# ironhide23586/RoomNet

Hardware: AMD Instinct MI355X
Metric: images/sec, 224x224 batch-256 RoomNet inference (higher is better)
Workload: dtype bf16; 1 GPU; RoomNet forward (reference final_model weights), uint8 BGR 224x224x3 in HBM -> probs+ids in HBM, batch 256 per GPU, bf16 storage / fp32 accumulate; images_per_gpu=256, global_batch=256, im_side=224, parallelism=dp1

## Files before the change

roomnet_amd/csrc/rn_fused.hip:

```cpp
#include "rn_fused.h"
#include <map>
#include <vector>
#include <algorithm>
#include <atomic>
#include "rn_stage.h"

#include <cmath>
#include <cstring>
#include <cstdlib>

using namespace rnk;

namespace {

constexpr int S0_CO = 8;
constexpr int S0_TSTRIDE = 29;
constexpr int S0_AHEAD = 8;

struct Stage0Args {
    const uint8_t* bgr;
    const i32x4* wfrag;
    const float* ptab;
    unsigned short* out;
    int S, So;
// ... 1123 lines not shown
            for (int b = 1; b <= 8 && b <= max_bands; ++b) {
                const long rounds = (per_band * b + n_cu - 1) / n_cu;
                const long cost = rounds * ((s2.out_side + b - 1) / b + 11);
                if (best_cost < 0 || cost < best_cost) {
                    best_cost = cost;
                    bands = b;
                }
            }
            if (per_band * bands < n_cu) {
                bands = static_cast<int>((n_cu + per_band - 1) / per_band);
                if (bands > max_bands) bands = max_bands;
            }
            fa.rows_per_band = (s2.out_side + bands - 1) / bands;
            fa.n_bands = (s2.out_side + fa.rows_per_band - 1) / fa.rows_per_band;
#ifdef RN_STAMPS
            static unsigned long long* stamp_host23 = nullptr;
            const size_t nwaves23 = static_cast<size_t>(fa.n_bands) * fa.n_cblocks * n * 8;
            if (!stamp_host23) (void)hipHostMalloc(reinterpret_cast<void**>(&stamp_host23), 16u << 20, 0);
            std::memset(stamp_host23, 0, nwaves23 * 96);
            fa.stamp_buf = stamp_host23;
#endif
#ifdef RN_CLOCK
            if (fs->pair_x16) fa.stamp_buf = rn_clock_region("stages 2+3", static_cast<size_t>(fa.n_bands) * fa.n_cblocks * n);
#endif
#ifdef RN_ROUND2_ARMS
            int rc = fs->pair_x16 ? rn_stage23x_launch(h->dtype, h->stream, fa, n) : rn_stage23_launch(h->dtype, h->stream, fa, n);
#else
            int rc = rn_stage23x_launch(h->dtype, h->stream, fa, n);
#endif
            if (rc != RN_OK) return rc;
#ifdef RN_STAMPS
            (void)hipStreamSynchronize(h->stream);
            {
                double wtot[8] = {0}, wbar[8] = {0}, wsteps[8] = {0};
                for (size_t k = 0; k < nwaves23; ++k) {
                    wtot[k & 7] += stamp_host23[k * 4];
                    wbar[k & 7] += stamp_host23[k * 4 + 2];
                    wsteps[k & 7] += stamp_host23[k * 4 + 3];
                }
                {
                    double seg[2][6] = {{0}, {0}};
                    double st[2] = {0, 0};
                    const unsigned long long* base = stamp_host23 + nwaves23 * 4;
                    for (size_t k = 0; k < nwaves23; ++k) {
                        const int role = (k & 7) < 4 ? 0 : 1;
                        st[role] += stamp_host23[k * 4 + 3];
                        for (int j = 0; j < 6; ++j) seg[role][j] += base[k * 8 + j];
                    }
                    fprintf(stderr, "[stamps]   producer segments (chain0 epi0 chain1 epi1): %.0f %.0f %.0f %.0f\n", seg[0][0] / st[0], seg[0][1] / st[0],
                            seg[0][2] / st[0], seg[0][3] / st[0]);
                    fprintf(stderr, "[stamps]   consumer segments (bookkeeping+own-fetch chain0 skip-wait epi0 chain1+epi1): %.0f %.0f %.0f %.0f %.0f\n", seg[1][0] / st[1],
                            seg[1][2] / st[1], seg[1][3] / st[1], seg[1][4] / st[1], seg[1][5] / st[1]);
                }
                for (int w8 = 0; w8 < 8; ++w8)
                    if (wsteps[w8] > 0)
                        fprintf(stderr, "[stamps] fused stages %zu+%zu wave %d (%s): cycles/step %.0f, of which barrier wait %.0f\n", i, i + 1, w8,
                                w8 < 4 ? "producer" : "consumer", wtot[w8] / wsteps[w8], wbar[w8] / wsteps[w8]);
            }
#endif
            rn_record_event(h, 2 + static_cast<int>(i) + 1);
            ++i;
            continue;
        }
        StageArgs a{};
        a.in = static_cast<const unsigned short*>(h->nodes[prev.node_bn2 >= 0 ? prev.node_bn2 : prev.node_bn].ptr);
        a.out = static_cast<unsigned short*>(h->nodes[s.node_bn2 >= 0 ? s.node_bn2 : s.node_bn].ptr);
        a.wfrag = f.wfrag;
        a.bn_mean = s.bn.mean;
        a.bn_inv = s.bn.inv;
        a.bn_beta = s.bn.beta;
        if (s.skip_stage >= 0) {
            const StagePlan& sk = h->stages[s.skip_stage];
            if (sk.node_bn2 >= 0) {
                rn_set_error("16-bit path: skip source with its own residual is not supported");
                return RN_E_INVALID;
            }
            a.skip = static_cast<const unsigned short*>(h->nodes[sk.node_bn].ptr);
            a.bn2_mean = s.bn2.mean;
            a.bn2_inv = s.bn2.inv;
            a.bn2_beta = s.bn2.beta;
            a.rlo = s.rt.lo;
            a.rhi = s.rt.hi;
            a.rlerp = s.rt.lerp;
            a.Ss = s.skip_side;
            a.rscale = static_cast<float>(s.skip_side) / static_cast<float>(s.out_side);
        }
        a.H = a.W = s.in_side;
        a.Ho = a.Wo = s.out_side;
        a.dither = fs->dither_out[i];
        a.plain_q = -1;
// ... 277 lines not shown
```

roomnet_amd/csrc/rn_stage23x.hip:

```cpp
#include "rn_fused.h"
#include "rn_stage.h"

#include <atomic>
#include <utility>

using namespace rnk;

namespace {

template <int DT>
__device__ __forceinline__ unsigned pack2p(float a, float b) {
    return pack2<DT>(a, b);
}

constexpr int RN_NT_OUT = 2, RN_NT_SKIP = 2;
constexpr int X_NA = 4, X_NB = 4, X_NSK = 3;
constexpr int X_WMIN = 193;
constexpr int X_WMAX = 215;
constexpr int X_ROWA = X_WMAX * 64;
constexpr int X_BDUMMY = X_WMAX - 5;
constexpr int X_ROWB = (X_BDUMMY + 1) * 64;
constexpr int X_SKROW = 64 * 64;
constexpr int X_ROWB_N = (X_BDUMMY + 1) * 32;
constexpr int X_ROWB_8 = (X_BDUMMY + 1) * 16;
constexpr int X_NTAB = 6 * 32;
constexpr int X_RINGA_OFF = 1024;
constexpr int X_RINGB_OFF = X_RINGA_OFF + X_NA * X_ROWA;
constexpr int X_SKIP_OFF = X_RINGB_OFF + X_NB * X_ROWB;
constexpr int X_LDS = X_SKIP_OFF + 4 * X_NSK * X_SKROW;
constexpr int X_LAG = 11;
constexpr int X_KT = 9;
static_assert(X_LDS <= 160 * 1024, "LDS budget");

__device__ __forceinline__ int xp_start(int w) { return w == 0 ? 0 : w == 1 ? 61 : w == 2 ? 122 : 167; }
__device__ __forceinline__ int xc_start(int w) { return w == 0 ? 0 : w == 1 ? 45 : w == 2 ? 90 : 148; }

__device__ __forceinline__ unsigned lds_addr(const void* p) {
    return static_cast<unsigned>(reinterpret_cast<uintptr_t>((__attribute__((address_space(3))) const char*)p));
}

__device__ __forceinline__ int swzx(int pix) { return (pix >> 1) & 3; }

using i32x2 = __attribute__((ext_vector_type(2))) int;

template <int DT>
__device__ __forceinline__ f32x4 mfma16(i32x4 a, i32x4 b, f32x4 c) {
    if constexpr (DT == RN_DTYPE_BF16)
        return __builtin_amdgcn_mfma_f32_16x16x32_bf16(__builtin_bit_cast(bf16x8, a), __builtin_bit_cast(bf16x8, b), c, 0, 0, 0);
    else
        return __builtin_amdgcn_mfma_f32_16x16x32_f16(__builtin_bit_cast(f16x8, a), __builtin_bit_cast(f16x8, b), c, 0, 0, 0);
}

template <int DT, int PH, bool NB, bool N8 = false>
__global__ __launch_bounds__(512, 2) void stage23x_kernel(const Stage23Args a) {
    static_assert(!NB || PH == 1, "the narrow B ring holds the computed half only");
    static_assert(!N8 || NB, "the eight-channel ring is a narrow ring");
    constexpr int ROWB = N8 ? X_ROWB_8 : NB ? X_ROWB_N : X_ROWB;
    constexpr int AHEAD = 3;
    extern __shared__ __attribute__((aligned(64))) char smem[];
    const int tid = threadIdx.x;
    const int lane = tid & 63;
    const int wave = __builtin_amdgcn_readfirstlane(tid >> 6);
    const int wq = wave & 3;
    const int px16 = lane & 15, g = lane >> 4;
#ifdef RN_CLOCK
    unsigned long long ck_t0, ck_r0;
    clock_pair(ck_t0, ck_r0);
#endif
    const int cblk = blockIdx.x % a.n_cblocks, band = blockIdx.x / a.n_cblocks, n = blockIdx.y;
    const int Win = a.W, Hout = a.Wo, x0 = a.cb_x0[cblk];
    const int Wo = a.cb_wo[cblk], W = Wo + 10, Wb = W - 5;
    const int yo0 = band * a.rows_per_band;
    const int nrows = min(Hout, yo0 + a.rows_per_band) - yo0;
    const int nsteps = nrows + X_LAG;

    float* const tab = reinterpret_cast<float*>(smem);
    for (int i = tid; i < X_NTAB; i += 512) tab[i] = a.ptab[i];
    char* const ringA = smem + X_RINGA_OFF;
    char* const ringB = smem + X_RINGB_OFF;
    const unsigned ringA_lds = lds_addr(ringA), ringB_lds = lds_addr(ringB);
    const char* const in_img = reinterpret_cast<const char*>(a.in + static_cast<int64_t>(n) * Win * Win * 32);
    const char* const in_blk = in_img + x0 * 64;
    constexpr int OOB = 0x40000000;
    const f32x4 zero4 = {0.f, 0.f, 0.f, 0.f};

    i32x4 pm, pmx;
#pragma unroll
    for (int d = 0; d < 4; ++d) {
        unsigned w0 = 0, w1 = 0;
#pragma unroll
        for (int e2 = 0; e2 < 2; ++e2) {
            const int e = 2 * d + e2;
            const int p = 4 * g + (e & 3);
            w0 |= ((p >= px16 && p < px16 + 4) ? 0x3C00u : 0u) << (16 * e2);
            w1 |= ((16 + p >= px16 && 16 + p < px16 + 4) ? 0x3C00u : 0u) << (16 * e2);
        }
        pm[d] = static_cast<int>(w0);
        pmx[d] = static_cast<int>(w1);
    }
    asm volatile("" : "+v"(pm), "+v"(pmx));

    auto chain = [&](auto S0C, auto ROWC, auto KC, const unsigned (&base)[3], const i32x4 (&wr)[2 * X_KT], f32x4 (&acc)[2], auto&& hook) __attribute__((always_inline)) {
        constexpr int S0 = decltype(S0C)::value, ROW = decltype(ROWC)::value, k = decltype(KC)::value;
        i32x4 fq[X_KT];
        auto rd = [&](auto TC, float dep) __attribute__((always_inline)) -> i32x4 {
            constexpr int tap = decltype(TC)::value, ky = tap / 3, kx = tap % 3;
            constexpr int off = ((S0 + ky) % 4) * ROW + k * 1024;
            i32x4 v;
            asm volatile("ds_read_b128 %0, %1 offset:%2" : "=v"(v) : "v"(base[kx]), "n"(off), "v"(dep));
            return v;
        };
        [&]<int... I>(std::integer_sequence<int, I...>) { ((fq[I] = rd(IC<I>{}, 0.f)), ...); }(std::make_integer_sequence<int, AHEAD>{});
// ... 17 lines not shown
        if constexpr (sub == 1) vt[h][1] = static_cast<int>(pack2_relu6_sixth(acc[h][2], acc[h][3]));
        if constexpr (sub == 2) {
            const int n0 = pk_add_f16(hp[h][0], vt[h][0]), n1 = pk_add_f16(hp[h][1], vt[h][1]);
            hp[h][0] = vt[h][0];
            hp[h][1] = vt[h][1];
            if constexpr (NB) {
                auto& Q = PR == 0 ? q0[h] : q1[h];
                Q[2 * HI] = n0;
                Q[2 * HI + 1] = n1;
                op[h] = Q;
            } else {
                auto& qold = PR == 0 ? q0[h] : q1[h];
                op[h] = i32x4{qold[0], qold[1], n0, n1};
                qold[0] = n0;
                qold[1] = n1;
            }
        }
    };
    auto finish = [&](auto PRC, const f32x4 (&acc)[2], int (&hp)[2][2], auto& q0, auto& q1, i32x4 (&op)[2]) __attribute__((always_inline)) {
        int vt[2][2];
        [&]<int... I>(std::integer_sequence<int, I...>) { (finish_part(IC<I>{}, PRC, acc, hp, q0, q1, op, vt), ...); }(std::make_integer_sequence<int, 6>{});
    };
    auto with_finish = [&](auto&& base, auto PRC, const f32x4 (&acc)[2], int (&hp)[2][2], auto& q0, auto& q1, i32x4 (&op)[2],
                           int (&vt)[2][2]) __attribute__((always_inline)) {
        return [&, PRC](auto IC_) __attribute__((always_inline)) {
            constexpr int i = decltype(IC_)::value;
            base(IC_);
            if constexpr (i >= 1 && i <= 6) finish_part(IC<(i >= 1 && i <= 6 ? i - 1 : 0)>{}, PRC, acc, hp, q0, q1, op, vt);
        };
    };

    const int xs0 = a.rlo[x0 + min(xc_start(wq), Wo - 1)];
    const unsigned sk_goff0 = static_cast<unsigned>((xs0 + (lane >> 2)) * 64 + ((lane & 3) << 4));
    char* const skw = smem + X_SKIP_OFF + wq * (X_NSK * X_SKROW);
    const unsigned skw_lds = lds_addr(skw);
    auto issue_skip_piece = [&](auto IC_, int y, int slot) __attribute__((always_inline)) {
        constexpr int i = decltype(IC_)::value;
        const char* row = in_img + static_cast<int64_t>(y) * static_cast<int64_t>(Win * 64);
        unsigned off = sk_goff0;
        asm volatile("" : "+v"(off));
        __builtin_amdgcn_global_load_lds(row + i * 1024 + off, (lds_void_ptr)(skw + slot * X_SKROW + i * 1024), 16, 0, RN_NT_SKIP);
    };
    auto issue_skip_row = [&](int y, int slot) __attribute__((always_inline)) {
        issue_skip_piece(IC<0>{}, y, slot);
        issue_skip_piece(IC<1>{}, y, slot);
        issue_skip_piece(IC<2>{}, y, slot);
        issue_skip_piece(IC<3>{}, y, slot);
    };
    auto no_hook = [](auto) __attribute__((always_inline)) {};
    struct VLerp {
        int ylo;
        float yl;
    };
    auto vlerp_of = [&](int yo) __attribute__((always_inline)) -> VLerp {
        const float src = mul_rounded(static_cast<float>(yo), a.rscale);
        const int ylo = static_cast<int>(src);
        VLerp v;
        v.ylo = __builtin_amdgcn_readfirstlane(ylo);
        v.yl = __int_as_float(__builtin_amdgcn_readfirstlane(__float_as_int(src - static_cast<float>(ylo))));
        return v;
    };
    int sk_f = vlerp_of(yo0).ylo - 1;
    int sk_slot = X_NSK - 1;
    auto ylo_step = [&](int t) __attribute__((always_inline)) {
        return vlerp_of(yo0 + min(max(t - X_LAG, 0), nrows - 1)).ylo;
    };

// ... 46 lines not shown
        for (int k = 0; k < 4; ++k) {
            const int xo = xw + 16 * k + px16;
            const bool last = k == (has4 ? 3 : 2);
            const int col = (xo < Wb && !(last && px16 >= 13) && (k < 3 || has4)) ? xo : X_BDUMMY;
            if constexpr (N8)
                wbB[k] = ringB_lds + static_cast<unsigned>((g < 2 ? col : X_BDUMMY) * 16 + 8 * (g & 1));
            else if constexpr (NB)
                wbB[k] = ringB_lds + static_cast<unsigned>(col * 32 + 8 * g);
            else
                wbB[k] = ringB_lds + static_cast<unsigned>(col * 64 + ((g ^ swzx(col)) << 4));
        }
        f32x4 scv[2], shv[2];
#pragma unroll
        for (int h = 0; h < 2; ++h) {
            scv[h] = *reinterpret_cast<const f32x4*>(a.ptab + 8 * g + 4 * h);
            shv[h] = *reinterpret_cast<const f32x4*>(a.ptab + 32 + 8 * g + 4 * h);
        }
        int hp[4][2][2];
        std::conditional_t<NB, i32x4[4][2], int[4][2][2]> q0, q1;
#pragma unroll
        for (int k = 0; k < 4; ++k)
#pragma unroll
            for (int h = 0; h < 2; ++h)
#pragma unroll
                for (int j = 0; j < 2; ++j) {
                    hp[k][h][j] = 0;
                    if constexpr (NB) {
                        q0[k][h][2 * j] = q0[k][h][2 * j + 1] = q1[k][h][2 * j] = q1[k][h][2 * j + 1] = 0;
                    } else {
                        q0[k][h][j] = q1[k][h][j] = 0;
                    }
                }
        issue_A_pieces(a_next, 0);
        int ylo_nxt = ylo_step(0);
        wait_vmcnt<0>();
#pragma unroll
        for (int f = 0; f < 2 * X_KT; ++f)
            if (PH == 2 || !(f & 1)) asm volatile("" : "+v"(w2[f]));
        lds_barrier();
        [[maybe_unused]] const int cdead0 = static_cast<int>(pack2p<DT>(shv[1][0], shv[1][1])), cdead1 = static_cast<int>(pack2p<DT>(shv[1][2], shv[1][3]));

        [[maybe_unused]] auto chain2 = [&](auto S0C, auto K0C, auto K1C, f32x4& acc0, f32x4& acc1, auto&& hook) __attribute__((always_inline)) {
            constexpr int S0 = decltype(S0C)::value, k0 = decltype(K0C)::value, k1 = decltype(K1C)::value;
            i32x4 fa[X_KT], fb[X_KT];
            auto rd = [&](auto TC, auto KC_, float dep) __attribute__((always_inline)) -> i32x4 {
                constexpr int tap = decltype(TC)::value, ky = tap / 3, kx = tap % 3, k = decltype(KC_)::value;
                constexpr int off = ((S0 + ky) % 4) * X_ROWA + k * 1024;
                i32x4 v;
                asm volatile("ds_read_b128 %0, %1 offset:%2" : "=v"(v) : "v"(baseA[kx]), "n"(off), "v"(dep));
                return v;
            };
            [&]<int... I>(std::integer_sequence<int, I...>) { ((fa[I] = rd(IC<I>{}, IC<k0>{}, 0.f), fb[I] = rd(IC<I>{}, IC<k1>{}, 0.f)), ...); }(std::make_integer_sequence<int, AHEAD>{});
            [&]<int... I>(std::integer_sequence<int, I...>) {
                (([&] {
                     if constexpr (I + AHEAD < X_KT) {
                         fa[I + AHEAD] = rd(IC<(I + AHEAD < X_KT ? I + AHEAD : 0)>{}, IC<k0>{}, I == 0 ? 0.f : acc0[0]);
                         fb[I + AHEAD] = rd(IC<(I + AHEAD < X_KT ? I + AHEAD : 0)>{}, IC<k1>{}, I == 0 ? 0.f : acc1[0]);
                     }
                     constexpr int newer = (X_KT - 1 - I) < AHEAD ? (X_KT - 1 - I) : AHEAD;
                     asm volatile("s_waitcnt lgkmcnt(%2)" : "+v"(fa[I]), "+v"(fb[I]) : "n"(2 * newer));
                     acc0 = mfma16<DT>(fa[I], w2[2 * I], I == 0 ? zero4 : acc0);
                     acc1 = mfma16<DT>(fb[I], w2[2 * I], I == 0 ? zero4 : acc1);
                     hook(IC<I>{});
                 }()),
                 ...);
            }(std::make_integer_sequence<int, X_KT>{});
        };
        [[maybe_unused]] auto chain1 = [&](auto S0C, auto KC_, f32x4& acc0, auto&& hook) __attribute__((always_inline)) {
            constexpr int S0 = decltype(S0C)::value, k = decltype(KC_)::value;
            i32x4 fa[X_KT];
            auto rd = [&](auto TC, float dep) __attribute__((always_inline)) -> i32x4 {
                constexpr int tap = decltype(TC)::value, ky = tap / 3, kx = tap % 3;
                constexpr int off = ((S0 + ky) % 4) * X_ROWA + k * 1024;
                i32x4 v;
                asm volatile("ds_read_b128 %0, %1 offset:%2" : "=v"(v) : "v"(baseA[kx]), "n"(off), "v"(dep));
                return v;
            };
            [&]<int... I>(std::integer_sequence<int, I...>) { ((fa[I] = rd(IC<I>{}, 0.f)), ...); }(std::make_integer_sequence<int, AHEAD>{});
            [&]<int... I>(std::integer_sequence<int, I...>) {
                (([&] {
                     if constexpr (I + AHEAD < X_KT) fa[I + AHEAD] = rd(IC<(I + AHEAD < X_KT ? I + AHEAD : 0)>{}, I == 0 ? 0.f : acc0[0]);
                     constexpr int newer = (X_KT - 1 - I) < AHEAD ? (X_KT - 1 - I) : AHEAD;
                     asm volatile("s_waitcnt lgkmcnt(%1)" : "+v"(fa[I]) : "n"(newer));
                     acc0 = mfma16<DT>(fa[I], w2[2 * I], I == 0 ? zero4 : acc0);
                     hook(IC<I>{});
                 }()),
                 ...);
            }(std::make_integer_sequence<int, X_KT>{});
        };
        [[maybe_unused]] auto with_finish2 = [&](auto&& base, auto PRC, const f32x4 (&accx)[2], int (&hpx)[2][2], auto& q0x, auto& q1x, i32x4 (&opx)[2],
                                const f32x4 (&accy)[2], int (&hpy)[2][2], auto& q0y, auto& q1y, i32x4 (&opy)[2], int (&vt)[2][2]) __attribute__((always_inline)) {
            return [&, PRC](auto IC_) __attribute__((always_inline)) {
                constexpr int i = decltype(IC_)::value;
                base(IC_);
                if constexpr (i >= 1 && i <= 3) finish_part(IC<(i >= 1 && i <= 3 ? i - 1 : 0)>{}, PRC, accx, hpx, q0x, q1x, opx, vt);
                if constexpr (i >= 4 && i <= 6) finish_part(IC<(i >= 4 && i <= 6 ? i - 4 : 0)>{}, PRC, accy, hpy, q0y, q1y, opy, vt);
            };
        };
        [[maybe_unused]] auto finish1 = [&](auto PRC, const f32x4 (&acc)[2], int (&hpx)[2][2], auto& q0x, auto& q1x, i32x4 (&opx)[2]) __attribute__((always_inline)) {
            int vt[2][2];
            finish_part(IC<0>{}, PRC, acc, hpx, q0x, q1x, opx, vt);
            finish_part(IC<1>{}, PRC, acc, hpx, q0x, q1x, opx, vt);
            finish_part(IC<2>{}, PRC, acc, hpx, q0x, q1x, opx, vt);
        };
        [[maybe_unused]] auto out1 = [&](auto KC, auto PC, const i32x4 (&opk)[2], const i32x4 (&opn)[2], bool cross) __attribute__((always_inline)) {
            constexpr int k = decltype(KC)::value, P = decltype(PC)::value;
            constexpr int off = ((P + 3) % X_NB) * ROWB;
            f32x4 H = mfma16<RN_DTYPE_F16>(opk[0], pm, zero4);
// ... 1 lines not shown
            float y[4];
#pragma unroll
            for (int i = 0; i < 4; ++i) y[i] = __builtin_fmaf(H[i], scv[0][i], shv[0][i]);
            auto& wb = wbB;
            if constexpr (NB) {
                const i32x2 d = {static_cast<int>(pack2p<DT>(y[0], y[1])), static_cast<int>(pack2p<DT>(y[2], y[3]))};
                asm volatile("ds_write_b64 %0, %1 offset:%2" ::"v"(wb[k]), "v"(d), "n"(off) : "memory");
            } else {
                const i32x4 d = {static_cast<int>(pack2p<DT>(y[0], y[1])), static_cast<int>(pack2p<DT>(y[2], y[3])), cdead0, cdead1};
                asm volatile("ds_write_b128 %0, %1 offset:%2" ::"v"(wb[k]), "v"(d), "n"(off) : "memory");
            }
        };

        auto out = [&](auto KC, auto PC, const i32x4 (&opk)[2], const i32x4 (&opn)[2], bool cross) __attribute__((always_inline)) {
            constexpr int k = decltype(KC)::value, P = decltype(PC)::value;
            constexpr int off = ((P + 3) % X_NB) * X_ROWB;
            f32x4 H[2];
#pragma unroll
            for (int h = 0; h < 2; ++h) H[h] = mfma16<RN_DTYPE_F16>(opk[h], pm, zero4);
            if (cross) {
#pragma unroll
                for (int h = 0; h < 2; ++h) H[h] = mfma16<RN_DTYPE_F16>(opn[h], pmx, H[h]);
            }
            float y[8];
#pragma unroll
            for (int h = 0; h < 2; ++h)
#pragma unroll
                for (int i = 0; i < 4; ++i) y[4 * h + i] = __builtin_fmaf(H[h][i], scv[h][i], shv[h][i]);
            const i32x4 d = {static_cast<int>(pack2p<DT>(y[0], y[1])), static_cast<int>(pack2p<DT>(y[2], y[3])),
                             static_cast<int>(pack2p<DT>(y[4], y[5])), static_cast<int>(pack2p<DT>(y[6], y[7]))};
            auto& wb = wbB;
            asm volatile("ds_write_b128 %0, %1 offset:%2" ::"v"(wb[k]), "v"(d), "n"(off) : "memory");
        };
        auto step = [&](auto PC, int t) __attribute__((always_inline)) {
            constexpr int P = decltype(PC)::value;
            [[maybe_unused]] constexpr int PR = P & 1;
            if (t < nrows + 9) a_next += Win * 64;
            auto hook0 = [&](auto IC_) __attribute__((always_inline)) {
                constexpr int i = decltype(IC_)::value;
                if constexpr (i == 1) issue_A_piece(IC<0>{}, a_next, (P + 1) % X_NA);
                if constexpr (i == 5) issue_A_piece(IC<1>{}, a_next, (P + 1) % X_NA);
                if constexpr (i == 3) {
                    const int need_cur = min(ylo_nxt + 1, Win - 1);
                    if (sk_f < need_cur) {
                        ++sk_f;
                        sk_slot = sk_slot == X_NSK - 1 ? 0 : sk_slot + 1;
                    }
                }
                if constexpr (i == 7) {
                    ylo_nxt = ylo_step(t + 1);
                    const int need_next = min(ylo_nxt + 1, Win - 1);
                    if (sk_f < need_next) {
                        ++sk_f;
                        sk_slot = sk_slot == X_NSK - 1 ? 0 : sk_slot + 1;
                    }
                }
            };
            auto hook1 = [&](auto IC_) __attribute__((always_inline)) {
                constexpr int i = decltype(IC_)::value;
                if constexpr (i == 1) issue_A_piece(IC<2>{}, a_next, (P + 1) % X_NA);
                if constexpr (i == 5) issue_A_piece(IC<3>{}, a_next, (P + 1) % X_NA);
            };
            auto hook2 = [&](auto IC_) __attribute__((always_inline)) {
                constexpr int i = decltype(IC_)::value;
                if constexpr (i == 0) issue_skip_piece(IC<0>{}, sk_f, sk_slot);
                if constexpr (i == 2) issue_skip_piece(IC<1>{}, sk_f, sk_slot);
                if constexpr (i == 4) issue_skip_piece(IC<2>{}, sk_f, sk_slot);
                if constexpr (i == 6) issue_skip_piece(IC<3>{}, sk_f, sk_slot);
            };
            if constexpr (PH == 1) {
                auto hookA = [&](auto IC_) __attribute__((always_inline)) {
                    constexpr int i = decltype(IC_)::value;
                    if constexpr (i == 0) issue_A_piece(IC<0>{}, a_next, (P + 1) % X_NA);
                    if constexpr (i == 2) issue_A_piece(IC<1>{}, a_next, (P + 1) % X_NA);
                    if constexpr (i == 4) issue_A_piece(IC<2>{}, a_next, (P + 1) % X_NA);
                    if constexpr (i == 6) issue_A_piece(IC<3>{}, a_next, (P + 1) % X_NA);
                    if constexpr (i == 3 || i == 7) hook0(IC_);
                };
                f32x4 ac0[2], ac1[2], ac2[2], ac3[2];
                int vt[2][2];
                i32x4 op[4][2];
                op[3][0] = op[3][1] = i32x4{0, 0, 0, 0};
                chain2(IC<(P + 2) % 4>{}, IC<0>{}, IC<1>{}, ac0[0], ac1[0], hookA);
                if (has4) {
                    chain2(IC<(P + 2) % 4>{}, IC<2>{}, IC<3>{}, ac2[0], ac3[0],
                           with_finish2(hook2, IC<(P & 3)>{}, ac0, hp[0], q0[0], q1[0], op[0], ac1, hp[1], q0[1], q1[1], op[1], vt));
                    out1(IC<0>{}, PC, op[0], op[1], true);
                    finish1(IC<(P & 3)>{}, ac2, hp[2], q0[2], q1[2], op[2]);
                    out1(IC<1>{}, PC, op[1], op[2], true);
                    finish1(IC<(P & 3)>{}, ac3, hp[3], q0[3], q1[3], op[3]);
                    out1(IC<2>{}, PC, op[2], op[3], true);
                    out1(IC<3>{}, PC, op[3], op[3], false);
                } else {
                    chain1(IC<(P + 2) % 4>{}, IC<2>{}, ac2[0],
                           with_finish2(hook2, IC<(P & 3)>{}, ac0, hp[0], q0[0], q1[0], op[0], ac1, hp[1], q0[1], q1[1], op[1], vt));
                    out1(IC<0>{}, PC, op[0], op[1], true);
                    finish1(IC<(P & 3)>{}, ac2, hp[2], q0[2], q1[2], op[2]);
                    out1(IC<1>{}, PC, op[1], op[2], true);
                    out1(IC<2>{}, PC, op[2], op[3], true);
                }
                wait_vmcnt<0>();
                asm volatile("s_waitcnt lgkmcnt(0)" ::: "memory");
                raw_barrier();
                return;
            }
            f32x4 accA[2], accB[2];
            int vt[2][2];
            i32x4 op[4][2];
            op[3][0] = op[3][1] = i32x4{0, 0, 0, 0};
            chain(IC<(P + 2) % 4>{}, IC<X_ROWA>{}, IC<0>{}, baseA, w2, accA, hook0);
            chain(IC<(P + 2) % 4>{}, IC<X_ROWA>{}, IC<1>{}, baseA, w2, accB, with_finish(hook1, IC<(P & 3)>{}, accA, hp[0], q0[0], q1[0], op[0], vt));
            chain(IC<(P + 2) % 4>{}, IC<X_ROWA>{}, IC<2>{}, baseA, w2, accA, with_finish(hook2, IC<(P & 3)>{}, accB, hp[1], q0[1], q1[1], op[1], vt));
            out(IC<0>{}, PC, op[0], op[1], true);
            if (has4) {
                chain(IC<(P + 2) % 4>{}, IC<X_ROWA>{}, IC<3>{}, baseA, w2, accB, with_finish(no_hook, IC<(P & 3)>{}, accA, hp[2], q0[2], q1[2], op[2], vt));
                out(IC<1>{}, PC, op[1], op[2], true);
                finish(IC<(P & 3)>{}, accB, hp[3], q0[3], q1[3], op[3]);
                out(IC<2>{}, PC, op[2], op[3], true);
                out(IC<3>{}, PC, op[3], op[3], false);
            } else {
                finish(IC<(P & 3)>{}, accA, hp[2], q0[2], q1[2], op[2]);
                out(IC<1>{}, PC, op[1], op[2], true);
                out(IC<2>{}, PC, op[2], op[3], true);
            }
            wait_vmcnt<0>();
            asm volatile("s_waitcnt lgkmcnt(0)" ::: "memory");
            raw_barrier();
        };
        int t = 0;
        for (; t + 3 < nsteps; t += 4) {
            step(IC<0>{}, t);
            step(IC<1>{}, t + 1);
            step(IC<2>{}, t + 2);
            step(IC<3>{}, t + 3);
        }
        const int rem = nsteps - t;
        if (rem > 0) step(IC<0>{}, t);
        if (rem > 1) step(IC<1>{}, t + 1);
        if (rem > 2) step(IC<2>{}, t + 2);
        wait_vmcnt<0>();
        return;
    }

    __builtin_amdgcn_s_setprio(1);
    const bool has4 = wq >= 2;
    const int xw = xc_start(wq);
    const int xend = wq == 3 ? Wo : min(xc_start(wq + 1), Wo);
    constexpr int NW3 = N8 ? 6 : NB ? 10 : 2 * X_KT;
    i32x4 w3[2 * X_KT];
#pragma unroll
    for (int f = 0; f < NW3; ++f) {
        const i32x4* src = a.wfrag3 + f * 64 + lane;
        asm volatile("global_load_dwordx4 %0, %1, off" : "=v"(w3[f]) : "v"(src) : "memory");
    }
    unsigned baseB[3], a_off[4];
    i32x4 wx[4];
#pragma unroll
    for (int kx = 0; kx < 3; ++kx) {
        const int p = xw + px16 + kx;
        baseB[kx] = ringB_lds + static_cast<unsigned>(p * 64 + ((g ^ swzx(p)) << 4));
    }
    [[maybe_unused]] unsigned baseN0 = 0, baseMix = 0, baseMixW = 0;
    [[maybe_unused]] f32x4 cinit[2] = {zero4, zero4};
    if constexpr (NB) {
        if constexpr (!N8) {
        const unsigned lane0 = ringB_lds + static_cast<unsigned>((xw + px16) * 32 + ((g & 1) << 4));
        baseN0 = lane0 + static_cast<unsigned>((g >> 1) * 32);
        baseMix = lane0 + static_cast<unsigned>((g >> 1) ? X_ROWB_N : 64);
        baseMixW = lane0 + static_cast<unsigned>((g >> 1) ? 0 : 3 * X_ROWB_N + 64);
        }
#pragma unroll
        for (int h = 0; h < 2; ++h) {
            const float c = a.ptab[160 + 8 * (px16 >> 2) + 4 * h + (px16 & 3)];
// ... 185 lines not shown
            const f32x4 r_hi = mfma16<DT>(ah, wx[k], zero4);
#pragma unroll
            for (int i = 0; i < 4; ++i) {
                const float y1 = __builtin_fmaf(H[h][i], tsc1[h][i], tsh1[h][i]);
                const float lo = r_lo[i];
                const float rs = __builtin_fmaf(r_hi[i] - lo, cx.yl, lo);
                y[4 * h + i] = __builtin_fmaf(rs, tsc2[h][i], y1);
            }

        }
        i32x4 d;
        if constexpr (DT == RN_DTYPE_BF16)
            d = i32x4{static_cast<int>(pack2_sr_bf16(y[0], y[1], cx.seed)), static_cast<int>(pack2_sr_bf16(y[2], y[3], cx.seed)),
                      static_cast<int>(pack2_sr_bf16(y[4], y[5], cx.seed)), static_cast<int>(pack2_sr_bf16(y[6], y[7], cx.seed))};
        else
            d = i32x4{static_cast<int>(pack2<DT>(y[0], y[1])), static_cast<int>(pack2<DT>(y[2], y[3])),
                      static_cast<int>(pack2<DT>(y[4], y[5])), static_cast<int>(pack2<DT>(y[6], y[7]))};
        const __amdgpu_buffer_rsrc_t rs = __builtin_amdgcn_make_buffer_rsrc(const_cast<char*>(cx.row), 0, out_row_bytes, 0x00020000);
        const int vo = (px16 < lim(k) ? voff0 + 1024 * k : OOB) | cx.emit_mask;
        __builtin_amdgcn_raw_buffer_store_b128(d, rs, vo, 0, RN_NT_OUT);
    };
    auto step = [&](auto PC, int t) __attribute__((always_inline)) {
        constexpr int P = decltype(PC)::value;
        [[maybe_unused]] constexpr int PR = P & 1;
        const int jo = t - X_LAG;
        cx.yl = vl_cur.yl;
        cx.sk_lo = static_cast<unsigned>(slot_cur * X_SKROW);
        cx.sk_hi = static_cast<unsigned>((vl_cur.ylo + 1 > Win - 1 ? slot_cur : (slot_cur == X_NSK - 1 ? 0 : slot_cur + 1)) * X_SKROW);
        cx.row = out_row;
        cx.emit_mask = jo >= 0 ? 0 : OOB;
        cx.seed = a.dither ? rn_dither_seed(yo0 + max(jo, 0)) : RN_SEED_PLAIN;
        if (jo >= 0 && jo < nrows - 1) out_row += out_row_bytes;
        const VLerp vl_next = vl_pre;
        {
            const int need_cur = min(vl_cur.ylo + 1, Win - 1);
            if (sk_f < need_cur) {
                ++sk_f;
                sk_slot = sk_slot == X_NSK - 1 ? 0 : sk_slot + 1;
                issue_skip_row(sk_f, sk_slot);
            }
            const int need_next = min(vl_next.ylo + 1, Win - 1);
            if (sk_f < need_next) {
                ++sk_f;
                sk_slot = sk_slot == X_NSK - 1 ? 0 : sk_slot + 1;
            }
        }
        f32x4 accA[2], accB[2];
        int vt[2][2];
        i32x4 op[4][2];
        op[3][0] = op[3][1] = i32x4{0, 0, 0, 0};
        OutRegs R;
        auto hook_c2 = [&](auto IC_) __attribute__((always_inline)) {
            if constexpr (decltype(IC_)::value == 7) vl_pre = vlerp_of(yo0 + min(max(jo + 2, 0), nrows - 1));
        };
        cchain(IC<P>{}, IC<0>{}, accA, no_hook);
        cchain(IC<P>{}, IC<1>{}, accB, with_finish(no_hook, IC<(P & 3)>{}, accA, hp[0], q0[0], q1[0], op[0], vt));
        wait_vmcnt<0>();
        out_reads(IC<0>{}, R);
        cchain(IC<P>{}, IC<2>{}, accA, with_finish(hook_c2, IC<(P & 3)>{}, accB, hp[1], q0[1], q1[1], op[1], vt));
        out_rest(IC<0>{}, R, op[0], op[1], true);
        if (has4) {
            out_reads(IC<1>{}, R);
            cchain(IC<P>{}, IC<3>{}, accB, with_finish(no_hook, IC<(P & 3)>{}, accA, hp[2], q0[2], q1[2], op[2], vt));
            out_rest(IC<1>{}, R, op[1], op[2], true);
            out_reads(IC<2>{}, R);
            finish(IC<(P & 3)>{}, accB, hp[3], q0[3], q1[3], op[3]);
            __builtin_amdgcn_sched_barrier(0);
            out_rest(IC<2>{}, R, op[2], op[3], true);
            out_reads(IC<3>{}, R);
            out_rest(IC<3>{}, R, op[3], op[3], false);
        } else {
            out_reads(IC<1>{}, R);
            finish(IC<(P & 3)>{}, accA, hp[2], q0[2], q1[2], op[2]);
            __builtin_amdgcn_sched_barrier(0);
            out_rest(IC<1>{}, R, op[1], op[2], true);
            out_reads(IC<2>{}, R);
            out_rest(IC<2>{}, R, op[2], op[3], true);
        }
        {
            int sl = slot_cur + (vl_next.ylo - vl_cur.ylo);
            slot_cur = sl >= X_NSK ? sl - X_NSK : sl;
            vl_cur = vl_next;
        }
        asm volatile("s_waitcnt lgkmcnt(0)" ::: "memory");
        raw_barrier();
    };
    int t = 0;
    for (; t + 3 < nsteps; t += 4) {
        step(IC<0>{}, t);
        step(IC<1>{}, t + 1);
        step(IC<2>{}, t + 2);
        step(IC<3>{}, t + 3);
    }
    const int rem = nsteps - t;
    if (rem > 0) step(IC<0>{}, t);
    if (rem > 1) step(IC<1>{}, t + 1);
    if (rem > 2) step(IC<2>{}, t + 2);
    wait_vmcnt<0>();
#ifdef RN_CLOCK
    if (a.stamp_buf && tid == 256) {
        unsigned long long t1, r1;
        clock_pair(t1, r1);
        const int64_t wg = static_cast<int64_t>(blockIdx.y) * gridDim.x + blockIdx.x;
        a.stamp_buf[wg * 2 + 0] = t1 - ck_t0;
        a.stamp_buf[wg * 2 + 1] = r1 - ck_r0;
    }
#endif
}

}

bool rn_stage23_plan(int in_side, int* n_cblocks, int* x0, int* wo) {
    const int out = in_side - 10;
    if (out < X_WMIN - 10) return false;
    const int nb = (out + (X_WMAX - 10) - 1) / (X_WMAX - 10);
    if (nb > 4) return false;
    const int base = out / nb, rem = out % nb;
    if (base + 10 < X_WMIN) return false;
    int x = 0;
    for (int b = 0; b < nb; ++b) {
        const int w = base + (b < rem ? 1 : 0);
        if (x0) x0[b] = x;
        if (wo) wo[b] = w;
        x += w;
    }
    if (n_cblocks) *n_cblocks = nb;
    return true;
}

bool rn_stage23_supported(int in_side) { return rn_stage23_plan(in_side, nullptr, nullptr, nullptr); }

// ... 11 lines not shown
}

void rn_stage23x_pack_narrow(const float* w_hwio, const int* ring_cin, int dtype, std::vector<unsigned short>* out) {
    out->assign(static_cast<size_t>(10) * 64 * 8, 0);
    for (int c = 0; c < 5; ++c)
        for (int h = 0; h < 2; ++h)
            for (int l = 0; l < 64; ++l)
                for (int jj = 0; jj < 8; ++jj) {
                    const int tap = 2 * c + (l >> 5), nn = l & 15;
                    if (tap > 8) continue;
                    const int cin = ring_cin[8 * ((l >> 4) & 1) + jj];
                    const int co = 8 * (nn >> 2) + 4 * h + (nn & 3);
                    const float v = w_hwio[(static_cast<size_t>(tap) * 32 + cin) * 32 + co];
                    (*out)[((static_cast<size_t>(c) * 2 + h) * 64 + l) * 8 + jj] = rn_to16(v, dtype);
                }
}

void rn_stage23x_pack_narrow8(const float* w_hwio, const int* ring_cin, int dtype, std::vector<unsigned short>* out) {
    out->assign(static_cast<size_t>(6) * 64 * 8, 0);
    for (int c = 0; c < 3; ++c)
        for (int h = 0; h < 2; ++h)
            for (int l = 0; l < 64; ++l)
                for (int jj = 0; jj < 8; ++jj) {
                    const int tap = 4 * c + (l >> 4), nn = l & 15;
                    if (tap > 8) continue;
                    const int cin = ring_cin[jj];
                    const int co = 8 * (nn >> 2) + 4 * h + (nn & 3);
                    const float v = w_hwio[(static_cast<size_t>(tap) * 32 + cin) * 32 + co];
                    (*out)[((static_cast<size_t>(c) * 2 + h) * 64 + l) * 8 + jj] = rn_to16(v, dtype);
                }
}

int rn_stage23x_launch(int dtype, hipStream_t s, const Stage23Args& a, int n) {
    auto launch = [&](auto kern) -> int {
        static std::atomic<unsigned long long> attr_devices{0};
        int dev = 0;
        RN_HIP(hipGetDevice(&dev));
        if (!(attr_devices.load(std::memory_order_acquire) >> (dev & 63) & 1ull)) {
            RN_HIP(hipFuncSetAttribute(reinterpret_cast<const void*>(kern), hipFuncAttributeMaxDynamicSharedMemorySize, 160 * 1024));
            attr_devices.fetch_or(1ull << (dev & 63), std::memory_order_release);
        }
        hipLaunchKernelGGL(kern, dim3(a.n_bands * a.n_cblocks, n), dim3(512), X_LDS, s, a);
        RN_CHECK_LAUNCH();
        return RN_OK;
    };
    if (a.producer_halves == 1 && a.narrow_b == 2) {
        if (dtype == RN_DTYPE_BF16) return launch(stage23x_kernel<RN_DTYPE_BF16, 1, true, true>);
        return launch(stage23x_kernel<RN_DTYPE_F16, 1, true, true>);
    }
    if (a.producer_halves == 1 && a.narrow_b) {
        if (dtype == RN_DTYPE_BF16) return launch(stage23x_kernel<RN_DTYPE_BF16, 1, true>);
        return launch(stage23x_kernel<RN_DTYPE_F16, 1, true>);
    }
    if (a.producer_halves == 1) {
        rn_set_error("stage23x: producer_halves == 1 runs in the narrow form only");
        return RN_E_STATE;
    }
    if (dtype == RN_DTYPE_BF16) return launch(stage23x_kernel<RN_DTYPE_BF16, 2, false>);
    return launch(stage23x_kernel<RN_DTYPE_F16, 2, false>);
}
```

Baseline: 236,700 images/sec.

## Deepen A and skip rings in narrow stage23x to keep loads in flight across barriers

For the single-producer-half narrow variant, the A ring grows from 4 to 5 rows and the skip ring from 3 to 4 slots. The prologue now prefetches two A rows, and each step waits only until four loads remain instead of draining all outstanding global loads before the barrier. The consumer skip fetch also moves earlier into the producer chain, and ring row offsets become runtime registers rather than compile-time constants. This is meant to hide global-load latency behind the per-step barrier, at the cost of more LDS per block (which may lower occupancy) and extra address arithmetic. Optional timing stamps and a median-based report are added for diagnostics.

```diff
diff --git a/roomnet_amd/csrc/rn_fused.hip b/roomnet_amd/csrc/rn_fused.hip
--- a/roomnet_amd/csrc/rn_fused.hip
+++ b/roomnet_amd/csrc/rn_fused.hip
@@ -1179,30 +1179,28 @@
 #ifdef RN_STAMPS
             (void)hipStreamSynchronize(h->stream);
             {
-                double wtot[8] = {0}, wbar[8] = {0}, wsteps[8] = {0};
+                std::vector<double> seg[2][3];
                 for (size_t k = 0; k < nwaves23; ++k) {
-                    wtot[k & 7] += stamp_host23[k * 4];
-                    wbar[k & 7] += stamp_host23[k * 4 + 2];
-                    wsteps[k & 7] += stamp_host23[k * 4 + 3];
-                }
-                {
-                    double seg[2][6] = {{0}, {0}};
-                    double st[2] = {0, 0};
-                    const unsigned long long* base = stamp_host23 + nwaves23 * 4;
-                    for (size_t k = 0; k < nwaves23; ++k) {
-                        const int role = (k & 7) < 4 ? 0 : 1;
-                        st[role] += stamp_host23[k * 4 + 3];
-                        for (int j = 0; j < 6; ++j) seg[role][j] += base[k * 8 + j];
+                    const unsigned long long* w = stamp_host23 + k * 4;
+                    if (!w[3]) continue;
+                    const double steps = static_cast<double>(w[3]);
+                    const int role = (k & 7) < 4 ? 0 : 1;
+                    seg[role][0].push_back(static_cast<double>(w[1]) / steps);
+                    seg[role][1].push_back(static_cast<double>(w[2]) / steps);
+                    seg[role][2].push_back(static_cast<double>(w[0] - w[1] - w[2]) / steps);
+                }
+                for (int role = 0; role < 2; ++role) {
+                    if (seg[role][0].empty()) continue;
+                    double med[3];
+                    for (int j = 0; j < 3; ++j) {
+                        std::sort(seg[role][j].begin(), seg[role][j].end());
+                        med[j] = seg[role][j][seg[role][j].size() / 2];
                     }
-                    fprintf(stderr, "[stamps]   producer segments (chain0 epi0 chain1 epi1): %.0f %.0f %.0f %.0f\n", seg[0][0] / st[0], seg[0][1] / st[0],
-                            seg[0][2] / st[0], seg[0][3] / st[0]);
-                    fprintf(stderr, "[stamps]   consumer segments (bookkeeping+own-fetch chain0 skip-wait epi0 chain1+epi1): %.0f %.0f %.0f %.0f %.0f\n", seg[1][0] / st[1],
-                            seg[1][2] / st[1], seg[1][3] / st[1], seg[1][4] / st[1], seg[1][5] / st[1]);
-                }
-                for (int w8 = 0; w8 < 8; ++w8)
-                    if (wsteps[w8] > 0)
-                        fprintf(stderr, "[stamps] fused stages %zu+%zu wave %d (%s): cycles/step %.0f, of which barrier wait %.0f\n", i, i + 1, w8,
-                                w8 < 4 ? "producer" : "consumer", wtot[w8] / wsteps[w8], wbar[w8] / wsteps[w8]);
+                    const double tot = med[0] + med[1] + med[2];
+                    fprintf(stderr, "[stamps] fused stages %zu+%zu %s waves (median of %zu): cycles per row step: vmcnt waits %.0f (%.1f %%), "
+                            "barrier %.0f (%.1f %%), rest %.0f (%.1f %%)\n", i, i + 1, role ? "consumer" : "producer", seg[role][0].size(),
+                            med[0], 100.0 * med[0] / tot, med[1], 100.0 * med[1] / tot, med[2], 100.0 * med[2] / tot);
+                }
             }
 #endif
             rn_record_event(h, 2 + static_cast<int>(i) + 1);
diff --git a/roomnet_amd/csrc/rn_stage23x.hip b/roomnet_amd/csrc/rn_stage23x.hip
--- a/roomnet_amd/csrc/rn_stage23x.hip
+++ b/roomnet_amd/csrc/rn_stage23x.hip
@@ -14,7 +14,7 @@
 }
 
 constexpr int RN_NT_OUT = 2, RN_NT_SKIP = 2;
-constexpr int X_NA = 4, X_NB = 4, X_NSK = 3;
+constexpr int X_NB = 4;
 constexpr int X_WMIN = 193;
 constexpr int X_WMAX = 215;
 constexpr int X_ROWA = X_WMAX * 64;
@@ -25,12 +25,20 @@
 constexpr int X_ROWB_8 = (X_BDUMMY + 1) * 16;
 constexpr int X_NTAB = 6 * 32;
 constexpr int X_RINGA_OFF = 1024;
-constexpr int X_RINGB_OFF = X_RINGA_OFF + X_NA * X_ROWA;
-constexpr int X_SKIP_OFF = X_RINGB_OFF + X_NB * X_ROWB;
-constexpr int X_LDS = X_SKIP_OFF + 4 * X_NSK * X_SKROW;
 constexpr int X_LAG = 11;
 constexpr int X_KT = 9;
-static_assert(X_LDS <= 160 * 1024, "LDS budget");
+
+template <int PH, bool NB, bool N8>
+struct XLayout {
+    static constexpr bool KEEP = PH == 1;
+    static constexpr int NA = KEEP ? 5 : 4;
+    static constexpr int NSK = KEEP ? 4 : 3;
+    static constexpr int ROWB = N8 ? X_ROWB_8 : NB ? X_ROWB_N : X_ROWB;
+    static constexpr int RINGB_OFF = X_RINGA_OFF + NA * X_ROWA;
+    static constexpr int SKIP_OFF = RINGB_OFF + X_NB * ROWB;
+    static constexpr int LDS = SKIP_OFF + 4 * NSK * X_SKROW;
+    static_assert(LDS <= 160 * 1024, "LDS budget");
+};
 
 __device__ __forceinline__ int xp_start(int w) { return w == 0 ? 0 : w == 1 ? 61 : w == 2 ? 122 : 167; }
 __device__ __forceinline__ int xc_start(int w) { return w == 0 ? 0 : w == 1 ? 45 : w == 2 ? 90 : 148; }
@@ -40,6 +48,16 @@
 }
 
 __device__ __forceinline__ int swzx(int pix) { return (pix >> 1) & 3; }
+
+#ifdef RN_STAMPS
+__device__ __forceinline__ unsigned long long stamp() {
+    unsigned long long t;
+    __builtin_amdgcn_sched_barrier(0);
+    asm volatile("s_memtime %0\n\ts_waitcnt lgkmcnt(0)" : "=s"(t)::"memory");
+    __builtin_amdgcn_sched_barrier(0);
+    return t;
+}
+#endif
 
 using i32x2 = __attribute__((ext_vector_type(2))) int;
 
@@ -55,7 +73,9 @@
 __global__ __launch_bounds__(512, 2) void stage23x_kernel(const Stage23Args a) {
     static_assert(!NB || PH == 1, "the narrow B ring holds the computed half only");
     static_assert(!N8 || NB, "the eight-channel ring is a narrow ring");
-    constexpr int ROWB = N8 ? X_ROWB_8 : NB ? X_ROWB_N : X_ROWB;
+    using L = XLayout<PH, NB, N8>;
+    constexpr bool KEEP = L::KEEP;
+    constexpr int ROWB = L::ROWB, X_NA = L::NA, X_NSK = L::NSK;
     constexpr int AHEAD = 3;
     extern __shared__ __attribute__((aligned(64))) char smem[];
     const int tid = threadIdx.x;
@@ -67,6 +87,36 @@
     unsigned long long ck_t0, ck_r0;
     clock_pair(ck_t0, ck_r0);
 #endif
+#ifdef RN_STAMPS
+    unsigned long long st_loop = 0, st_wait = 0, st_bar = 0, st_steps = 0;
+    auto stamps_out = [&]() __attribute__((always_inline)) {
+        if (a.stamp_buf && lane == 0) {
+            const int64_t w = (static_cast<int64_t>(blockIdx.y) * gridDim.x + blockIdx.x) * 8 + wave;
+            a.stamp_buf[w * 4 + 0] = st_loop;
+            a.stamp_buf[w * 4 + 1] = st_wait;
+            a.stamp_buf[w * 4 + 2] = st_bar;
+            a.stamp_buf[w * 4 + 3] = st_steps;
+        }
+    };
+#endif
+    auto close_step = [&](auto VMC) __attribute__((always_inline)) {
+        constexpr int VM = decltype(VMC)::value;
+#ifdef RN_STAMPS
+        const unsigned long long ts1 = stamp();
+#endif
+        if constexpr (VM >= 0) wait_vmcnt<(VM >= 0 ? VM : 0)>();
+#ifdef RN_STAMPS
+        const unsigned long long ts2 = stamp();
+#endif
+        asm volatile("s_waitcnt lgkmcnt(0)" ::: "memory");
+        raw_barrier();
+#ifdef RN_STAMPS
+        const unsigned long long ts3 = stamp();
+        st_wait += ts2 - ts1;
+        st_bar += ts3 - ts2;
+        ++st_steps;
+#endif
+    };
     const int cblk = blockIdx.x % a.n_cblocks, band = blockIdx.x / a.n_cblocks, n = blockIdx.y;
     const int Win = a.W, Hout = a.Wo, x0 = a.cb_x0[cblk];
     const int Wo = a.cb_wo[cblk], W = Wo + 10, Wb = W - 5;
@@ -77,7 +127,7 @@
     float* const tab = reinterpret_cast<float*>(smem);
     for (int i = tid; i < X_NTAB; i += 512) tab[i] = a.ptab[i];
     char* const ringA = smem + X_RINGA_OFF;
-    char* const ringB = smem + X_RINGB_OFF;
+    char* const ringB = smem + L::RINGB_OFF;
     const unsigned ringA_lds = lds_addr(ringA), ringB_lds = lds_addr(ringB);
     const char* const in_img = reinterpret_cast<const char*>(a.in + static_cast<int64_t>(n) * Win * Win * 32);
     const char* const in_blk = in_img + x0 * 64;
@@ -161,7 +211,7 @@
 
     const int xs0 = a.rlo[x0 + min(xc_start(wq), Wo - 1)];
     const unsigned sk_goff0 = static_cast<unsigned>((xs0 + (lane >> 2)) * 64 + ((lane & 3) << 4));
-    char* const skw = smem + X_SKIP_OFF + wq * (X_NSK * X_SKROW);
+    char* const skw = smem + L::SKIP_OFF + wq * (X_NSK * X_SKROW);
     const unsigned skw_lds = lds_addr(skw);
     auto issue_skip_piece = [&](auto IC_, int y, int slot) __attribute__((always_inline)) {
         constexpr int i = decltype(IC_)::value;
@@ -274,22 +324,26 @@
                     }
                 }
         issue_A_pieces(a_next, 0);
-        int ylo_nxt = ylo_step(0);
-        wait_vmcnt<0>();
+        if constexpr (KEEP) {
+            a_next += Win * 64;
+            issue_A_pieces(a_next, 1);
+        }
+        int ylo_nxt = ylo_step(KEEP ? 1 : 0);
+        wait_vmcnt<KEEP ? 4 : 0>();
 #pragma unroll
         for (int f = 0; f < 2 * X_KT; ++f)
             if (PH == 2 || !(f & 1)) asm volatile("" : "+v"(w2[f]));
         lds_barrier();
         [[maybe_unused]] const int cdead0 = static_cast<int>(pack2p<DT>(shv[1][0], shv[1][1])), cdead1 = static_cast<int>(pack2p<DT>(shv[1][2], shv[1][3]));
 
-        [[maybe_unused]] auto chain2 = [&](auto S0C, auto K0C, auto K1C, f32x4& acc0, f32x4& acc1, auto&& hook) __attribute__((always_inline)) {
-            constexpr int S0 = decltype(S0C)::value, k0 = decltype(K0C)::value, k1 = decltype(K1C)::value;
+        [[maybe_unused]] unsigned rowA[3] = {0, 0, 0};
+        [[maybe_unused]] auto chain2 = [&](auto K0C, auto K1C, f32x4& acc0, f32x4& acc1, auto&& hook) __attribute__((always_inline)) {
+            constexpr int k0 = decltype(K0C)::value, k1 = decltype(K1C)::value;
             i32x4 fa[X_KT], fb[X_KT];
             auto rd = [&](auto TC, auto KC_, float dep) __attribute__((always_inline)) -> i32x4 {
                 constexpr int tap = decltype(TC)::value, ky = tap / 3, kx = tap % 3, k = decltype(KC_)::value;
-                constexpr int off = ((S0 + ky) % 4) * X_ROWA + k * 1024;
                 i32x4 v;
-                asm volatile("ds_read_b128 %0, %1 offset:%2" : "=v"(v) : "v"(baseA[kx]), "n"(off), "v"(dep));
+                asm volatile("ds_read_b128 %0, %1 offset:%2" : "=v"(v) : "v"(baseA[kx] + rowA[ky]), "n"(k * 1024), "v"(dep));
                 return v;
             };
             [&]<int... I>(std::integer_sequence<int, I...>) { ((fa[I] = rd(IC<I>{}, IC<k0>{}, 0.f), fb[I] = rd(IC<I>{}, IC<k1>{}, 0.f)), ...); }(std::make_integer_sequence<int, AHEAD>{});
@@ -308,14 +362,13 @@
                  ...);
             }(std::make_integer_sequence<int, X_KT>{});
         };
-        [[maybe_unused]] auto chain1 = [&](auto S0C, auto KC_, f32x4& acc0, auto&& hook) __attribute__((always_inline)) {
-            constexpr int S0 = decltype(S0C)::value, k = decltype(KC_)::value;
+        [[maybe_unused]] auto chain1 = [&](auto KC_, f32x4& acc0, auto&& hook) __attribute__((always_inline)) {
+            constexpr int k = decltype(KC_)::value;
             i32x4 fa[X_KT];
             auto rd = [&](auto TC, float dep) __attribute__((always_inline)) -> i32x4 {
                 constexpr int tap = decltype(TC)::value, ky = tap / 3, kx = tap % 3;
-                constexpr int off = ((S0 + ky) % 4) * X_ROWA + k * 1024;
                 i32x4 v;
-                asm volatile("ds_read_b128 %0, %1 offset:%2" : "=v"(v) : "v"(baseA[kx]), "n"(off), "v"(dep));
+                asm volatile("ds_read_b128 %0, %1 offset:%2" : "=v"(v) : "v"(baseA[kx] + rowA[ky]), "n"(k * 1024), "v"(dep));
                 return v;
             };
             [&]<int... I>(std::integer_sequence<int, I...>) { ((fa[I] = rd(IC<I>{}, 0.f)), ...); }(std::make_integer_sequence<int, AHEAD>{});
@@ -383,10 +436,11 @@
             auto& wb = wbB;
             asm volatile("ds_write_b128 %0, %1 offset:%2" ::"v"(wb[k]), "v"(d), "n"(off) : "memory");
         };
+        [[maybe_unused]] int ra = X_NA - 2;
         auto step = [&](auto PC, int t) __attribute__((always_inline)) {
             constexpr int P = decltype(PC)::value;
             [[maybe_unused]] constexpr int PR = P & 1;
-            if (t < nrows + 9) a_next += Win * 64;
+            if (t < nrows + (KEEP ? 8 : 9)) a_next += Win * 64;
             auto hook0 = [&](auto IC_) __attribute__((always_inline)) {
                 constexpr int i = decltype(IC_)::value;
                 if constexpr (i == 1) issue_A_piece(IC<0>{}, a_next, (P + 1) % X_NA);
@@ -420,22 +474,36 @@
                 if constexpr (i == 6) issue_skip_piece(IC<3>{}, sk_f, sk_slot);
             };
             if constexpr (PH == 1) {
+                const int need_next = min(ylo_nxt + 1, Win - 1);
+                if (sk_f + 1 < need_next) {
+                    ++sk_f;
+                    sk_slot = sk_slot == X_NSK - 1 ? 0 : sk_slot + 1;
+                    issue_skip_row(sk_f, sk_slot);
+                }
+                if (sk_f < need_next) {
+                    ++sk_f;
+                    sk_slot = sk_slot == X_NSK - 1 ? 0 : sk_slot + 1;
+                }
+                const int slot_new = ra == 0 ? X_NA - 1 : ra - 1;
+#pragma unroll
+                for (int ky = 0; ky < 3; ++ky) rowA[ky] = static_cast<unsigned>((ra + ky >= X_NA ? ra + ky - X_NA : ra + ky) * X_ROWA);
+                auto hookS = [&](auto IC_) __attribute__((always_inline)) {
+                    constexpr int i = decltype(IC_)::value;
+                    if constexpr (i == 0 || i == 2 || i == 4 || i == 6) issue_skip_piece(IC<(i >> 1)>{}, sk_f, sk_slot);
+                    if constexpr (i == 7) ylo_nxt = ylo_step(t + 2);
+                };
                 auto hookA = [&](auto IC_) __attribute__((always_inline)) {
                     constexpr int i = decltype(IC_)::value;
-                    if constexpr (i == 0) issue_A_piece(IC<0>{}, a_next, (P + 1) % X_NA);
-                    if constexpr (i == 2) issue_A_piece(IC<1>{}, a_next, (P + 1) % X_NA);
-                    if constexpr (i == 4) issue_A_piece(IC<2>{}, a_next, (P + 1) % X_NA);
-                    if constexpr (i == 6) issue_A_piece(IC<3>{}, a_next, (P + 1) % X_NA);
-                    if constexpr (i == 3 || i == 7) hook0(IC_);
+                    if constexpr (i == 0 || i == 2 || i == 4 || i == 6) issue_A_piece(IC<(i >> 1)>{}, a_next, slot_new);
                 };
                 f32x4 ac0[2], ac1[2], ac2[2], ac3[2];
                 int vt[2][2];
                 i32x4 op[4][2];
                 op[3][0] = op[3][1] = i32x4{0, 0, 0, 0};
-                chain2(IC<(P + 2) % 4>{}, IC<0>{}, IC<1>{}, ac0[0], ac1[0], hookA);
+                chain2(IC<0>{}, IC<1>{}, ac0[0], ac1[0], hookS);
                 if (has4) {
-                    chain2(IC<(P + 2) % 4>{}, IC<2>{}, IC<3>{}, ac2[0], ac3[0],
-                           with_finish2(hook2, IC<(P & 3)>{}, ac0, hp[0], q0[0], q1[0], op[0], ac1, hp[1], q0[1], q1[1], op[1], vt));
+                    chain2(IC<2>{}, IC<3>{}, ac2[0], ac3[0],
+                           with_finish2(hookA, IC<(P & 3)>{}, ac0, hp[0], q0[0], q1[0], op[0], ac1, hp[1], q0[1], q1[1], op[1], vt));
                     out1(IC<0>{}, PC, op[0], op[1], true);
                     finish1(IC<(P & 3)>{}, ac2, hp[2], q0[2], q1[2], op[2]);
                     out1(IC<1>{}, PC, op[1], op[2], true);
@@ -443,16 +511,15 @@
                     out1(IC<2>{}, PC, op[2], op[3], true);
                     out1(IC<3>{}, PC, op[3], op[3], false);
                 } else {
-                    chain1(IC<(P + 2) % 4>{}, IC<2>{}, ac2[0],
-                           with_finish2(hook2, IC<(P & 3)>{}, ac0, hp[0], q0[0], q1[0], op[0], ac1, hp[1], q0[1], q1[1], op[1], vt));
+                    chain1(IC<2>{}, ac2[0],
+                           with_finish2(hookA, IC<(P & 3)>{}, ac0, hp[0], q0[0], q1[0], op[0], ac1, hp[1], q0[1], q1[1], op[1], vt));
                     out1(IC<0>{}, PC, op[0], op[1], true);
                     finish1(IC<(P & 3)>{}, ac2, hp[2], q0[2], q1[2], op[2]);
                     out1(IC<1>{}, PC, op[1], op[2], true);
                     out1(IC<2>{}, PC, op[2], op[3], true);
                 }
-                wait_vmcnt<0>();
-                asm volatile("s_waitcnt lgkmcnt(0)" ::: "memory");
-                raw_barrier();
+                close_step(IC<4>{});
+                ra = ra == X_NA - 1 ? 0 : ra + 1;
                 return;
             }
             f32x4 accA[2], accB[2];
@@ -474,10 +541,11 @@
                 out(IC<1>{}, PC, op[1], op[2], true);
                 out(IC<2>{}, PC, op[2], op[3], true);
             }
-            wait_vmcnt<0>();
-            asm volatile("s_waitcnt lgkmcnt(0)" ::: "memory");
-            raw_barrier();
-        };
+            close_step(IC<0>{});
+        };
+#ifdef RN_STAMPS
+        const unsigned long long st_loop0 = stamp();
+#endif
         int t = 0;
         for (; t + 3 < nsteps; t += 4) {
             step(IC<0>{}, t);
@@ -489,7 +557,13 @@
         if (rem > 0) step(IC<0>{}, t);
         if (rem > 1) step(IC<1>{}, t + 1);
         if (rem > 2) step(IC<2>{}, t + 2);
+#ifdef RN_STAMPS
+        st_loop = stamp() - st_loop0;
+#endif
         wait_vmcnt<0>();
+#ifdef RN_STAMPS
+        stamps_out();
+#endif
         return;
     }
 
@@ -741,7 +815,7 @@
         cx.seed = a.dither ? rn_dither_seed(yo0 + max(jo, 0)) : RN_SEED_PLAIN;
         if (jo >= 0 && jo < nrows - 1) out_row += out_row_bytes;
         const VLerp vl_next = vl_pre;
-        {
+        if constexpr (!KEEP) {
             const int need_cur = min(vl_cur.ylo + 1, Win - 1);
             if (sk_f < need_cur) {
                 ++sk_f;
@@ -764,7 +838,15 @@
         };
         cchain(IC<P>{}, IC<0>{}, accA, no_hook);
         cchain(IC<P>{}, IC<1>{}, accB, with_finish(no_hook, IC<(P & 3)>{}, accA, hp[0], q0[0], q1[0], op[0], vt));
-        wait_vmcnt<0>();
+        if constexpr (!KEEP) {
+#ifdef RN_STAMPS
+            const unsigned long long tw1 = stamp();
+#endif
+            wait_vmcnt<0>();
+#ifdef RN_STAMPS
+            st_wait += stamp() - tw1;
+#endif
+        }
         out_reads(IC<0>{}, R);
         cchain(IC<P>{}, IC<2>{}, accA, with_finish(hook_c2, IC<(P & 3)>{}, accB, hp[1], q0[1], q1[1], op[1], vt));
         out_rest(IC<0>{}, R, op[0], op[1], true);
@@ -791,9 +873,11 @@
             slot_cur = sl >= X_NSK ? sl - X_NSK : sl;
             vl_cur = vl_next;
         }
-        asm volatile("s_waitcnt lgkmcnt(0)" ::: "memory");
-        raw_barrier();
-    };
+        close_step(IC<-1>{});
+    };
+#ifdef RN_STAMPS
+    const unsigned long long st_loop0 = stamp();
+#endif
     int t = 0;
     for (; t + 3 < nsteps; t += 4) {
         step(IC<0>{}, t);
@@ -805,7 +889,13 @@
     if (rem > 0) step(IC<0>{}, t);
     if (rem > 1) step(IC<1>{}, t + 1);
     if (rem > 2) step(IC<2>{}, t + 2);
+#ifdef RN_STAMPS
+    st_loop = stamp() - st_loop0;
+#endif
     wait_vmcnt<0>();
+#ifdef RN_STAMPS
+    stamps_out();
+#endif
 #ifdef RN_CLOCK
     if (a.stamp_buf && tid == 256) {
         unsigned long long t1, r1;
@@ -883,7 +973,7 @@
 }
 
 int rn_stage23x_launch(int dtype, hipStream_t s, const Stage23Args& a, int n) {
-    auto launch = [&](auto kern) -> int {
+    auto launch = [&](auto kern, int lds) -> int {
         static std::atomic<unsigned long long> attr_devices{0};
         int dev = 0;
         RN_HIP(hipGetDevice(&dev));
@@ -891,22 +981,25 @@
             RN_HIP(hipFuncSetAttribute(reinterpret_cast<const void*>(kern), hipFuncAttributeMaxDynamicSharedMemorySize, 160 * 1024));
             attr_devices.fetch_or(1ull << (dev & 63), std::memory_order_release);
         }
-        hipLaunchKernelGGL(kern, dim3(a.n_bands * a.n_cblocks, n), dim3(512), X_LDS, s, a);
+        hipLaunchKernelGGL(kern, dim3(a.n_bands * a.n_cblocks, n), dim3(512), lds, s, a);
         RN_CHECK_LAUNCH();
         return RN_OK;
     };
     if (a.producer_halves == 1 && a.narrow_b == 2) {
-        if (dtype == RN_DTYPE_BF16) return launch(stage23x_kernel<RN_DTYPE_BF16, 1, true, true>);
-        return launch(stage23x_kernel<RN_DTYPE_F16, 1, true, true>);
+        constexpr int lds = XLayout<1, true, true>::LDS;
+        if (dtype == RN_DTYPE_BF16) return launch(stage23x_kernel<RN_DTYPE_BF16, 1, true, true>, lds);
+        return launch(stage23x_kernel<RN_DTYPE_F16, 1, true, true>, lds);
     }
     if (a.producer_halves == 1 && a.narrow_b) {
-        if (dtype == RN_DTYPE_BF16) return launch(stage23x_kernel<RN_DTYPE_BF16, 1, true>);
-        return launch(stage23x_kernel<RN_DTYPE_F16, 1, true>);
+        constexpr int lds = XLayout<1, true, false>::LDS;
+        if (dtype == RN_DTYPE_BF16) return launch(stage23x_kernel<RN_DTYPE_BF16, 1, true>, lds);
+        return launch(stage23x_kernel<RN_DTYPE_F16, 1, true>, lds);
     }
     if (a.producer_halves == 1) {
         rn_set_error("stage23x: producer_halves == 1 runs in the narrow form only");
         return RN_E_STATE;
     }
-    if (dtype == RN_DTYPE_BF16) return launch(stage23x_kernel<RN_DTYPE_BF16, 2, false>);
-    return launch(stage23x_kernel<RN_DTYPE_F16, 2, false>);
+    constexpr int lds = XLayout<2, false, false>::LDS;
+    if (dtype == RN_DTYPE_BF16) return launch(stage23x_kernel<RN_DTYPE_BF16, 2, false>, lds);
+    return launch(stage23x_kernel<RN_DTYPE_F16, 2, false>, lds);
 }
```

New measurement: 239,300 images/sec, median of 6. 1.1% higher.
